# gyuhyun-lee/offline_raytracer

Hardware: AMD Instinct MI355X
Metric: Mpaths/s (higher is better)
Workload: dtype f32; 1 GPU; c3_bunny_room.scn (69451 triangles) 1920x1080 1024spp rr0.8, CHUNK policy chunk=64, one frame sharded in 8x8 blocks over 1 GPU(s); width=1920, height=1080, spp=1024, gather=none (1 GPU): un-permute kernel only, gather_fallback=False, launch=single process, workspace_bytes_per_rank=398131200

## Files before the change

### offline_raytracer_amd/csrc/ort_kernels.hip

```cpp
#include <algorithm>
#include <type_traits>

#include "ort_lane.h"
#include "ort_plan.h"
#include "ort_setup.h"

#ifndef ORT_HOST_SIM
void ort_launch_w5(int diffuse, unsigned int grid, void *stream, const void *sv_bytes, const void *hot_bytes);
size_t ort_w5_sizeof_scene_view();
size_t ort_w5_sizeof_render_hot();
void ort_launch_radiance_adaptive(int counters, int diffuse, int tabs, unsigned int grid, void *stream, const void *sv_bytes, const void *hot_bytes);
size_t ort_adaptive_sizeof_scene_view();
size_t ort_adaptive_sizeof_render_hot();
size_t ort_adaptive_sizeof_render_view();

namespace ort {

using namespace ortd;

static_assert(kPlanBlock == (uint32_t)kBlock && kPlanLdsStack == (uint32_t)kLdsStack && kPlanStashVecs == kStashVecs && kPlanCapL == kCapL &&
              kPlanCapR == kCapR && (int)PLAN_JOBS_EXPLICIT == (int)JOBS_EXPLICIT &&
              (int)PLAN_JOBS_PIXEL == (int)JOBS_PIXEL && (int)PLAN_JOBS_CHUNK == (int)JOBS_CHUNK,
              "ort_plan.h counts with the lane code's limits");

// ... 353 lines not shown
        fprintf(stderr, "  %g ms: %zu", m, n);
    }
    fprintf(stderr, "\n");
    return ORT_OK;
}

static int print_util_diag(const DeviceScene *d, std::string *err) {
    static const char *names[8] = {"node visit", "leaf visit", "traverse outer iteration", "shade call", "  of which lanes with a finished ray",
                                   "produce_ray pass", "  bounce draw", "  sin/cos + ray setup"};
    unsigned long long u[16];
    ORT_HIP(hipMemcpy(u, d->ctrl() + 8, sizeof(u), hipMemcpyDeviceToHost));
    for (int k = 0; k < 8; ++k)
        fprintf(stderr, "util %-40s wave-events %14llu  mean active lanes %6.2f\n", names[k], u[2 * k],
                u[2 * k] ? (double)u[2 * k + 1] / (double)u[2 * k] : 0.0);
    static const char *pnames[10] = {"resolve_hit (chain check)", "hit processing + bounce draw", "pixel / job / new sample", "sin/cos + normalise + ray setup",
                                    "1/d + analytic prologue", "descend loop", "leaf", "pt_lane loop top (after traverse)",
                                    "produce_ray entry (after resolve)", "traverse loop top"};
    unsigned long long ph[30];
    ORT_HIP(hipMemcpy(ph, d->ctrl() + 8 + 32, sizeof(ph), hipMemcpyDeviceToHost));
    double total = 0;
    for (int k = 0; k < 10; ++k) total += (double)ph[3 * k];
    for (int k = 0; k < 10; ++k)
        fprintf(stderr, "phase %-36s share %5.1f %%  cycles/mark %8.1f  marks %12llu  lanes at mark %5.1f\n", pnames[k],
                total > 0 ? 100.0 * (double)ph[3 * k] / total : 0.0, ph[3 * k + 1] ? (double)ph[3 * k] / (double)ph[3 * k + 1] : 0.0,
                ph[3 * k + 1], ph[3 * k + 1] ? (double)ph[3 * k + 2] / (double)ph[3 * k + 1] : 0.0);
    return ORT_OK;
}

static int read_render_stats(const DeviceScene *d, bool counters, ort_stats *stats, std::string *err) {
    memset(stats, 0, sizeof(*stats));
    float ms = 0;
    ORT_HIP(hipEventElapsedTime(&ms, d->ev0, d->ev1));
    stats->kernel_ms = ms;
    unsigned long long c[6];
    ORT_HIP(hipMemcpy(c, d->ctrl() + 1, sizeof(c), hipMemcpyDeviceToHost));
    stats->fallback_rays = c[5];
    if (counters) { stats->paths = c[0]; stats->rays = c[1]; stats->node_tests = c[2]; stats->tri_tests = c[3]; stats->analytic_tests = c[4]; }
    return ORT_OK;
}

int device_render(Scene *scene, const ort_render_params *p, const ort_tile_job *jobs, uint32_t job_count, void *d_out,
                  float *h_out, void *stream_v, uint32_t *final_states, ort_stats *stats, std::string *err, const ort_view *views,
                  uint32_t view_count) {
    DeviceScene *d = scene->dev;
    if (!d) { *err = "scene is not uploaded to a device (ort_scene_upload)"; return ORT_ERR_NO_DEVICE; }
    ORT_HIP(hipSetDevice(d->device));
    hipStream_t stream = (hipStream_t)stream_v;
    const bool packed_out = (p->flags & ORT_RENDER_PACKED) != 0 && !jobs;
    if (!views) view_count = 1;
    const size_t image_bytes = packed_out ? (size_t)block_grid_for(p).my_blocks * 768u : (size_t)view_count * (size_t)p->width * (size_t)p->height * 12u;
    int rc;
    if ((rc = settle_inflight(d, err))) return rc;

    float *out = (float *)d_out;
    if (!out) {
        if ((rc = d->staging.ensure(image_bytes, err))) return rc;
        out = d->staging.as<float>();
        if (h_out) ORT_HIP(hipMemcpyAsync(out, h_out, image_bytes, hipMemcpyHostToDevice, stream));
    }

    SceneView sv = scene_view(scene, d);
    const bool w5_layout_ok = ort_w5_sizeof_scene_view() == sizeof(SceneView) && ort_w5_sizeof_render_hot() == sizeof(RenderHot);
    const LaunchPlan pl = plan_render(scene_traits(scene, d), *p, jobs != nullptr, job_count, w5_layout_ok, d->knobs, view_count);

    sv.util = pl.util ? d->ctrl() + 8 : nullptr;
    if (pl.wide) sv.nodes = d->nodes4.as<const float4>();
    ort_camera cam;
    camera_basis(*scene, p->width, p->height, &cam);
    if (views && !pl.views) cam = views[0].camera;
    memcpy(sv.cam, &cam, sizeof(cam));

    RenderView rv{};
    rv.W = p->width; rv.H = p->height;
    rv.x0 = p->x0; rv.y0 = p->y0; rv.x1 = p->x1; rv.y1 = p->y1;
    rv.seed = views && !pl.views ? views[0].seed : p->seed; rv.spp = p->spp; rv.chunk = p->chunk; rv.rr = p->rr;
    rv.out = out;
    rv.packed_out = packed_out;
    rv.next_job = d->ctrl();
    rv.counters = d->ctrl() + 1;
    rv.mode = pl.mode; rv.nchunks = pl.nchunks; rv.job_count = pl.job_count;
    rv.shard_count = pl.blocks.shard_count; rv.shard_index = pl.blocks.shard_index;
    rv.blocks_w = pl.blocks.blocks_w; rv.block_x0 = pl.blocks.block_x0; rv.block_y0 = pl.blocks.block_y0;
    rv.my_blocks = pl.blocks.my_blocks;
    rv.refill_below = pl.refill_below; rv.descend_below = pl.descend_below;
    rv.capL = pl.capL; rv.capR = pl.capR;
    rv.long_min = pl.long_min; rv.long_refill = pl.long_refill; rv.inflight_cap = pl.inflight_cap; rv.park_min = pl.park_min;
    rv.endgame_from = pl.endgame_from;
    rv.stash_wave_f4 = pl.stash_wave_f4;
    rv.block_major = pl.block_major;
    rv.job_batch = pl.job_batch; rv.batch_until = pl.batch_until;

    if (jobs) {
        if ((rc = d->jobs.ensure((size_t)job_count * sizeof(ort_tile_job), err))) return rc;
        ORT_HIP(hipStreamSynchronize(stream));
        ORT_HIP(hipMemcpy(d->jobs.p, jobs, (size_t)job_count * sizeof(ort_tile_job), hipMemcpyHostToDevice));
        rv.jobs = d->jobs.as<const ort_tile_job>();
        if (final_states) {
            if ((rc = d->states.ensure((size_t)job_count * 4u, err))) return rc;
            rv.final_states = d->states.as<uint32_t>();
        }
    }
    if (pl.views) {
        std::vector<float> &tab = d->view_tab_host;
        pack_view_table(views, view_count, tab);
        if ((rc = d->view_tab.ensure(tab.size() * sizeof(float), err))) return rc;
        ORT_HIP(hipMemcpyAsync(d->view_tab.p, tab.data(), tab.size() * sizeof(float), hipMemcpyHostToDevice, stream));
        rv.views = d->view_tab.as<const float4>();
        rv.view_jobs = pl.view_jobs;
        rv.view_count = pl.view_count;
    }
    if (pl.mode == PLAN_JOBS_CHUNK) {
        if ((rc = d->partial.ensure(pl.partial_bytes, err))) return rc;
        rv.partial = d->partial.as<float>();
    }
    if (pl.exchange) {
        if ((rc = d->stash.ensure(pl.stash_bytes, err))) return rc;
        rv.stash = d->stash.as<float4>();
    }
    ORT_HIP(hipMemsetAsync(d->ctrl(), 0, 128 * sizeof(unsigned long long), stream));
    if (pl.drain_bytes && stats) {
        if ((rc = d->drain.ensure(pl.drain_bytes, err))) return rc;
        ORT_HIP(hipMemsetAsync(d->drain.p, 0, pl.drain_bytes, stream));
        rv.drain = d->drain.as<unsigned long long>();
    }
    ORT_HIP(hipMemcpyAsync(d->rv_dev.p, &rv, sizeof(RenderView), hipMemcpyHostToDevice, stream));
    const RenderHot hot = render_hot<RenderHot>(rv, d->rv_dev.p);
    if (stats) ORT_HIP(hipEventRecord(d->ev0, stream));
    if (pl.wavefront) rc = pl.counters ? launch_wavefront<true>(d, sv, rv, hot, stream, err) : launch_wavefront<false>(d, sv, rv, hot, stream, err);
    else rc = launch_path_tracer(pl, stream, sv, hot, err);
    if (rc) return rc;
    ORT_HIP(hipGetLastError());
    if (rv.mode == JOBS_CHUNK) {
        unsigned long long total = (unsigned long long)rv.my_blocks * 64ull;
        unsigned int cgrid = (unsigned int)((total + 255) / 256);
        if (pl.views) {
            cgrid = (unsigned int)((total * pl.view_count + 255) / 256);
            if (cgrid) hipLaunchKernelGGL(combine_chunks_views, dim3(cgrid), dim3(256), 0, stream, hot);
        } else if (cgrid) hipLaunchKernelGGL(combine_chunks, dim3(cgrid), dim3(256), 0, stream, hot);
        ORT_HIP(hipGetLastError());
    }
    if (stats) ORT_HIP(hipEventRecord(d->ev1, stream));

    if (!d_out && h_out) ORT_HIP(hipMemcpyAsync(h_out, out, image_bytes, hipMemcpyDeviceToHost, stream));
    if (final_states) ORT_HIP(hipMemcpyAsync(final_states, d->states.p, (size_t)job_count * 4u, hipMemcpyDeviceToHost, stream));
    ORT_HIP(hipEventRecord(d->ev_done, stream));
    d->inflight = true;
    if (stats || !d_out || final_states)
        if ((rc = settle_inflight(d, err, "reference-order fallback queue overflowed"))) return rc;
    if (stats && d->knobs.debug_fallback && (rc = print_fallback_diag(d, pl, err))) return rc;
    if (stats && rv.drain && (rc = print_drain_diag(d, pl, err))) return rc;
    if (stats && (rc = read_render_stats(d, pl.counters, stats, err))) return rc;
    if (stats && pl.counters && pl.util && (rc = print_util_diag(d, err))) return rc;
    return ORT_OK;
}

constexpr uint64_t kRaycastSlice = 1ull << 22;
constexpr uint64_t kRadianceSlice = 1ull << 20;

static int ensure_prim_src(Scene *scene, DeviceScene *d, std::string *err) {
    if (d->prim_src.p) return ORT_OK;
    std::vector<uint32_t> src;
    const bool bijective = invert_prim_slots(scene->tree, d->info_box, d->info_cyl, d->info_sphere, src);
    if (!bijective) { *err = "internal: the tree's slot maps are not a bijection onto its shape arrays"; return ORT_ERR_INTERNAL; }
    return upload_vec(src, &d->prim_src, err);
}

static RaycastIO ray_query_io(Scene *scene, DeviceScene *d, const void *d_rays) {
// ... 187 lines not shown
```

### offline_raytracer_amd/csrc/ort_lane.h

```cpp
#ifndef ORT_LANE_H
#define ORT_LANE_H

#include <hip/hip_runtime.h>

#include <math.h>
#include <stdio.h>
#include <stdlib.h>
#include <string.h>

#include <algorithm>
#include <string>
#include <vector>

#include "ort_device.h"
#include "ort_scene.h"
#include "ort_setup.h"

#ifdef ORT_W5_TU
#define ORT_NS ort_w5
#elif defined(ORT_ADAPTIVE_TU)
#define ORT_NS ort_ad
#else
#define ORT_NS ort
#endif
// ... 33 lines not shown
    uint32_t bfs_queue_cap, bfs_queue_count;
    unsigned long long *fallback_counters;
};

struct PrimInfo { uint32_t chain, mat; };

struct SceneView {
    const float4 *tab_src;
    uint32_t tab_flags;
    const float4 *nodes;
    const float4 *tris;
    const float4 *spheres;
    const float4 *boxes;
    const float4 *cyls;
    const PrimInfo *prim_info;
    uint32_t info_box, info_cyl, info_sphere;
    const float4 *materials;
    const uint32_t *light_is_sphere;
    uint32_t light_count;
    uint32_t pro_boxes, pro_spheres, pro_cyls;
    float cam[12];
    const float4 *chain_boxes;
    const ORT_CONSTANT_AS SceneCold *cold;
    unsigned long long *util;
    uint32_t force_fallback_mask;
};

inline void build_prim_info(const Tree &t, const RefTree &rt, std::vector<PrimInfo> &out, uint32_t &info_box, uint32_t &info_cyl, uint32_t &info_sphere) {
    info_box = (uint32_t)t.tri_mat.size();
    info_cyl = info_box + (uint32_t)t.box_mat.size();
    info_sphere = info_cyl + (uint32_t)t.cyl_mat.size();
    out.assign((size_t)info_sphere + t.sphere_mat.size(), PrimInfo{0u, 0u});
    auto fill = [&out](uint32_t base, const std::vector<uint32_t> &chain, const std::vector<uint32_t> &mat) {
        for (size_t i = 0; i < mat.size(); ++i) out[base + i] = PrimInfo{i < chain.size() ? chain[i] : 0u, mat[i]};
    };
    fill(0u, rt.tri_chain, t.tri_mat);
    fill(info_box, rt.box_chain, t.box_mat);
    fill(info_cyl, rt.cyl_chain, t.cyl_mat);
    fill(info_sphere, rt.sphere_chain, t.sphere_mat);
}

enum : int { JOBS_EXPLICIT = 0, JOBS_PIXEL = 1, JOBS_CHUNK = 2 };

struct RenderView {
    int mode;
    const ort_tile_job *jobs;
    uint32_t *final_states;
    unsigned long long job_count;
    int W, H, x0, y0, x1, y1;
    uint32_t seed, spp, chunk, nchunks;
    float rr;
    int refill_below;
    int descend_below;
    uint32_t shard_index, shard_count, blocks_w, my_blocks;
    uint32_t block_x0, block_y0;
    float *out;
    float *partial;
    int packed_out;
    unsigned long long *next_job;
    unsigned long long *counters;
    float4 *stash;
    uint32_t stash_wave_f4;
    uint32_t capL, capR;
    uint32_t long_min;
    uint32_t long_refill;
    uint32_t park_min;
    uint32_t inflight_cap;
    uint32_t block_major;
    unsigned long long endgame_from;
    uint32_t job_batch;
    unsigned long long batch_until;
    unsigned long long *drain;
    const float4 *views;
    unsigned long long view_jobs;
    uint32_t view_count;
    const float2 *rays;
    const uint32_t *seeds;
    uint32_t ray_tree_spheres, ray_tree_quadrics, ray_tree_boxes;
    float ray_lo[3], ray_hi[3];
    uint32_t ad_min_spp, ad_check_every;
    float ad_tolerance, ad_floor;
    uint32_t *ad_spp;
    float *ad_m2;
};


struct RenderHot {
    int mode, W, H;
    float rr;
    int refill_below, descend_below;
    const ORT_CONSTANT_AS RenderView *c;
};

struct WfView {
    uint32_t slots;
    float4 *od0;
    float2 *od1;
    float4 *hit0;
    uint32_t *hitp;
    float4 *p0;
    float4 *p1;
    float4 *p2;
    uint4 *p3;
    uint32_t *flags;
    unsigned long long *active;
};

enum : int { PS_NEED_JOB = 0, PS_PIXEL = 1, PS_SAMPLE = 2, PS_HIT = 3, PS_DONE = 4 };

#ifdef ORT_HOST_SIM
#define ORT_BALLOT(p) ((p) ? 1ull : 0ull)
#define ORT_POPC64(m) __builtin_popcountll(m)
#define ORT_NEXT_JOB(p) __atomic_fetch_add((p), 1ull, __ATOMIC_RELAXED)
#define ORT_COUNT(p, v) ((void)__atomic_fetch_add((p), (v), __ATOMIC_RELAXED))
#define ORT_TRY_LOCK(p) (*(p) == 0u ? (*(p) = 1u, true) : false)
#define ORT_PEEK(p) (*(p))
#define ORT_BACKOFF()
#define ORT_UNLOCK(p) (*(p) = 0u)
#define ORT_FENCE()
#define ORT_FFS64(m) __builtin_ffsll((long long)(m))
#define ORT_LANE() 0
#define ORT_UTIL(sv, k, pred)
#define ORT_PHASE(pr, sv, k, pred)
#ifndef ORT_SIM_PIXEL_HOOK
#define ORT_SIM_PIXEL_HOOK(x, y, rng)
#endif
#ifndef ORT_SIM_RAY_HOOK
#define ORT_SIM_RAY_HOOK(x, y, o, d, t, n, m)
#endif
#else
#define ORT_SIM_PIXEL_HOOK(x, y, rng)
#define ORT_SIM_RAY_HOOK(x, y, o, d, t, n, m)
#define ORT_BALLOT(p) __ballot(p)
#define ORT_POPC64(m) __popcll(m)
#define ORT_NEXT_JOB(p) atomicAdd((p), 1ull)
#define ORT_COUNT(p, v) atomicAdd((p), (v))
#define ORT_TRY_LOCK(p) (atomicCAS((p), 0u, 1u) == 0u)
#define ORT_PEEK(p) __hip_atomic_load((p), __ATOMIC_RELAXED, __HIP_MEMORY_SCOPE_AGENT)
#define ORT_BACKOFF() __builtin_amdgcn_s_sleep(64)
#define ORT_UNLOCK(p) ((void)atomicExch((p), 0u))
#define ORT_FENCE() __threadfence()
#define ORT_FFS64(m) __ffsll((unsigned long long)(m))
#define ORT_LANE() ((int)__lane_id())
#define ORT_UTIL(sv, k, pred)                                                                        \
    do {                                                                                             \
        if (COUNTERS && (sv).util && blockIdx.x < 32u) {                                             \
            unsigned long long m_ = __ballot(pred);                                                  \
            if (m_ && (int)__lane_id() == __ffsll(m_) - 1) {                                         \
                atomicAdd(&g_lds_prof[2 * (k)], 1ull);                                               \
                atomicAdd(&g_lds_prof[2 * (k) + 1], (unsigned long long)__popcll(m_));               \
            }                                                                                        \
        }                                                                                            \
    } while (0)
#define ORT_PHASE(pr, sv, k, pred)                                                                   \
    do {                                                                                             \
        if (COUNTERS && (pr).on) {                                                                   \
            const unsigned long long now_ = __builtin_amdgcn_s_memtime();                            \
            const unsigned long long m_ = __ballot(pred), a_ = __ballot(true);                       \
             \
            unsigned long long *last_ = &g_lds_prof[96 + (threadIdx.x >> 6)];                        \
            if ((int)__lane_id() == __ffsll(a_) - 1) {                                               \
                atomicAdd(&g_lds_prof[32 + 3 * (k)], now_ - *last_);                                 \
                atomicAdd(&g_lds_prof[32 + 3 * (k) + 1], 1ull);                                      \
                atomicAdd(&g_lds_prof[32 + 3 * (k) + 2], (unsigned long long)__popcll(m_));          \
                *last_ = __builtin_amdgcn_s_memtime();                                               \
            }                                                                                        \
// ... 888 lines not shown
    float t0y = (a.y - org.y) * inv_d.y, t1y = (b.x - org.y) * inv_d.y;
    float t0z = (a.z - org.z) * inv_d.z, t1z = (b.y - org.z) * inv_d.z;
    float n0 = fmaxf(fmaxf(fminf(t0x, t1x), fminf(t0y, t1y)), fminf(t0z, t1z));
    float f0 = fminf(fminf(fmaxf(t0x, t1x), fmaxf(t0y, t1y)), fmaxf(t0z, t1z));
    float u0x = (b.z - org.x) * inv_d.x, u1x = (cc.y - org.x) * inv_d.x;
    float u0y = (b.w - org.y) * inv_d.y, u1y = (cc.z - org.y) * inv_d.y;
    float u0z = (cc.x - org.z) * inv_d.z, u1z = (cc.w - org.z) * inv_d.z;
    float n1 = fmaxf(fmaxf(fminf(u0x, u1x), fminf(u0y, u1y)), fminf(u0z, u1z));
    float f1 = fminf(fminf(fmaxf(u0x, u1x), fmaxf(u0y, u1y)), fmaxf(u0z, u1z));
    bool h0 = (f0 * 1.0000004f >= n0) && (f0 >= 0.0f) && ((n0 * kCullSlack < best_t) || (c0 & SPHERE_BELOW_BIT));
    bool h1 = (f1 * 1.0000004f >= n1) && (f1 >= 0.0f) && ((n1 * kCullSlack < best_t) || (c1 & SPHERE_BELOW_BIT)) && (c1 != EMPTY_CHILD);
    if (h0 && h1) {
        bool swap = n1 < n0;
        uint32_t farc = swap ? c0 : c1;
        cur = swap ? c1 : c0;
        if (sp < LDS_ENTRIES) lds_stack[sp * BLOCK + tid] = farc;
        else spill[sp - LDS_ENTRIES] = farc;
        sp++;
    } else if (h0) {
        cur = c0;
    } else if (h1) {
        cur = c1;
    } else if (sp == 0) {
        cur = kTraversalDone;
    } else {
        sp--;
        if (sp < LDS_ENTRIES) cur = lds_stack[sp * BLOCK + tid];
        else cur = ((volatile uint32_t *)spill)[sp - LDS_ENTRIES];
    }
}

template <bool COUNTERS, int LDS_ENTRIES, int BLOCK>
ORT_D void visit_node4(float4 lx, float4 ly, float4 lz, float4 hx, float4 hy, float4 hz, float4 cw, V3 org, V3 inv_d, float best_t, uint32_t &cur, int &sp,
                       uint32_t *lds_stack, uint32_t *spill, int tid, Counters &c) {
    if (COUNTERS) c.nodes += 4;
    float key0, key1, key2, key3;
    uint32_t w0, w1, w2, w3;
#define ORT_SLAB4(K, W, LX, LY, LZ, HX, HY, HZ, CW)                                                                        \
    {                                                                                                                      \
        const float t0x = ((LX) - org.x) * inv_d.x, t1x = ((HX) - org.x) * inv_d.x;                                        \
        const float t0y = ((LY) - org.y) * inv_d.y, t1y = ((HY) - org.y) * inv_d.y;                                        \
        const float t0z = ((LZ) - org.z) * inv_d.z, t1z = ((HZ) - org.z) * inv_d.z;                                        \
        const float n_ = fmaxf(fmaxf(fminf(t0x, t1x), fminf(t0y, t1y)), fminf(t0z, t1z));                                  \
        const float f_ = fminf(fminf(fmaxf(t0x, t1x), fmaxf(t0y, t1y)), fmaxf(t0z, t1z));                                  \
        const uint32_t cw_ = om_f32_bits(CW);                                                                              \
        const bool hit_ = (f_ * 1.0000004f >= n_) && (f_ >= 0.0f) && ((n_ * kCullSlack < best_t) || (cw_ & SPHERE_BELOW_BIT)) && (cw_ != EMPTY_CHILD); \
        K = hit_ ? fminf(n_, 3.402823466e+38f) : __builtin_inff();              \
        W = hit_ ? cw_ : EMPTY_CHILD;                                                                                      \
    }
    ORT_SLAB4(key0, w0, lx.x, ly.x, lz.x, hx.x, hy.x, hz.x, cw.x)
    ORT_SLAB4(key1, w1, lx.y, ly.y, lz.y, hx.y, hy.y, hz.y, cw.y)
    ORT_SLAB4(key2, w2, lx.z, ly.z, lz.z, hx.z, hy.z, hz.z, cw.z)
    ORT_SLAB4(key3, w3, lx.w, ly.w, lz.w, hx.w, hy.w, hz.w, cw.w)
#undef ORT_SLAB4
#define ORT_CX(KA, WA, KB, WB)                                                                                             \
    {                                                                                                                      \
        const bool sw_ = KB < KA;                                                                                          \
        const float ka_ = sw_ ? KB : KA, kb_ = sw_ ? KA : KB;                                                              \
        const uint32_t wa_ = sw_ ? WB : WA, wb_ = sw_ ? WA : WB;                                                           \
        KA = ka_; KB = kb_; WA = wa_; WB = wb_;                                                                            \
    }
    ORT_CX(key0, w0, key1, w1)
    ORT_CX(key2, w2, key3, w3)
    ORT_CX(key0, w0, key2, w2)
    ORT_CX(key1, w1, key3, w3)
    ORT_CX(key1, w1, key2, w2)
#undef ORT_CX
    if (w0 == EMPTY_CHILD) {
        if (sp == 0) {
            cur = kTraversalDone;
        } else {
            sp--;
            if (sp < LDS_ENTRIES) cur = lds_stack[sp * BLOCK + tid];
            else cur = ((volatile uint32_t *)spill)[sp - LDS_ENTRIES];
        }
        return;
    }
    cur = w0;
    if (w3 != EMPTY_CHILD) { if (sp < LDS_ENTRIES) lds_stack[sp * BLOCK + tid] = w3; else spill[sp - LDS_ENTRIES] = w3; sp++; }
    if (w2 != EMPTY_CHILD) { if (sp < LDS_ENTRIES) lds_stack[sp * BLOCK + tid] = w2; else spill[sp - LDS_ENTRIES] = w2; sp++; }
    if (w1 != EMPTY_CHILD) { if (sp < LDS_ENTRIES) lds_stack[sp * BLOCK + tid] = w1; else spill[sp - LDS_ENTRIES] = w1; sp++; }
}

template <bool COUNTERS, bool TABS, int LDS_ENTRIES, int BLOCK>
ORT_D void begin_ray(const SceneView &sv, const float4 *tab, const PathState &P, Trav &T, HitState &h, Counters &c, Prof &pr,
                     uint32_t *lds_stack, uint32_t *spill, int tid) {
    T.cur = 0;
    T.sp = 0;
    T.inv_d = mk(1.0f / P.dir.x, 1.0f / P.dir.y, 1.0f / P.dir.z);
    reset_hit(h, 3.402823466e+38f);
    prologue_tests<COUNTERS, TABS>(sv, tab, P.org, P.dir, T.inv_d, h, c);
    ORT_PHASE(pr, sv, 4, true);
}

template <bool COUNTERS, int LDS_ENTRIES, int BLOCK, bool TREELET = false, bool ANNOUNCE = false, bool WIDE = false>
ORT_D bool traverse(const SceneView &sv, V3 org, V3 dir, Trav &T, HitState &h, uint32_t *lds_stack, uint32_t *spill, int tid,
                    int refill_below, int descend_below, Counters &c, Prof &pr, uint32_t excl = kNoPrim, const float4 *tab = nullptr) {
    bool tracing = true;
    uint32_t cur = T.cur;
    int sp = T.sp;
    const V3 inv_d = T.inv_d;
    while (tracing) {
        ORT_UTIL(sv, 2, true);
        ORT_PHASE(pr, sv, 9, true);
        const int entering = ORT_POPC64(ORT_BALLOT((cur & LEAF_BIT) == 0u));
        const int stragglers = descend_below < (entering >> ORT_DESCEND_SHIFT) ? descend_below : (entering >> ORT_DESCEND_SHIFT);
        while (!(cur & LEAF_BIT)) {
            ORT_UTIL(sv, 0, true);
            const uint32_t ni = cur & NODE_INDEX_MASK;
            if (WIDE) {
                const float4 *np = sv.nodes + 8u * ni;
                const float4 lx = np[0], ly = np[1], lz = np[2], hx = np[3], hy = np[4], hz = np[5], cw = np[6];
                visit_node4<COUNTERS, LDS_ENTRIES, BLOCK>(lx, ly, lz, hx, hy, hz, cw, org, inv_d, h.best_t, cur, sp, lds_stack, spill, tid, c);
            } else {
            float4 na, nb, nc, nd;
            if (TREELET && ni < kTreeletNodes) {
                const float4 *np = tab + kTabTreelet + 4u * ni;
                na = np[0]; nb = np[1]; nc = np[2]; nd = np[3];
            } else {
                const float4 *np = sv.nodes + 4u * ni;
                na = np[0]; nb = np[1]; nc = np[2]; nd = np[3];
            }
            visit_node<COUNTERS, LDS_ENTRIES, BLOCK>(na, nb, nc, nd, org, inv_d, h.best_t, cur, sp, lds_stack, spill, tid, c);
            }
            if (ORT_POPC64(ORT_BALLOT(true)) < stragglers) break;
        }
        ORT_PHASE(pr, sv, 5, true);
        if (!(cur & LEAF_BIT)) {
        } else if (cur == kTraversalDone) {
            tracing = false;
        } else {
            ORT_UTIL(sv, 1, true);
            uint32_t kind = (cur >> 28) & 7u, count = ((cur >> 24) & 15u) + 1u, first = cur & 0x00ffffffu;
            for (uint32_t i = 0; i < count; ++i)
                test_prim<COUNTERS, false>(sv, kind, first + i, org, dir, inv_d, h.best_t, h.hit_n, h.hit_prim, h.phantom_t, h.runner_t, c.tris, c.analytic, excl);
            if (sp == 0) {
                cur = kTraversalDone;
                tracing = false;
            } else {
                sp--;
                if (sp < LDS_ENTRIES) cur = lds_stack[sp * BLOCK + tid];
                else cur = ((volatile uint32_t *)spill)[sp - LDS_ENTRIES];
            }
            ORT_PHASE(pr, sv, 6, true);
        }
        if (ANNOUNCE && !tracing) announce_winner<BLOCK>(sv, h.hit_prim, lds_stack, tid);
        if (refill_below > 0 && ORT_POPC64(ORT_BALLOT(tracing)) < refill_below) break;
    }
    T.cur = cur;
    T.sp = sp;
    return tracing;
}

template <bool COUNTERS, bool TABS, int LDS_ENTRIES, int BLOCK, bool ANNOUNCED = false, bool WIDE = false>
ORT_D void resolve_hit(const SceneView &sv, const float4 *tab, V3 org, V3 dir, V3 inv_d, uint32_t lane_id, HitState &h, Counters &c, Prof &pr,
                       uint32_t *lds_stack, uint32_t *spill, int tid) {
    uint32_t word = 0, mat = 0;
    if (ANNOUNCED) {
        announced_info<BLOCK>(lds_stack, tid, word, mat);
    } else if (h.hit_prim != kNoPrim) {
        const PrimInfo pi = sv.prim_info[info_index(sv, h.hit_prim)];
        word = pi.chain; mat = pi.mat;
    }
    bool stale = false;
    bool recast = sv.force_fallback_mask != 0xffffffffu && (om_f32_bits(dir.x) & sv.force_fallback_mask) == 0u;
    if (!ORT_RARE(recast)) {
        if (ORT_RARE(h.phantom_t <= h.best_t)) {
            recast = true;
            ORT_STAT(2, 1);
        } else if (h.hit_prim != kNoPrim) {
            float gap = 0.0f;
            const int verdict = chain_verdict(sv, word, org, inv_d, h.best_t, fminf(h.runner_t, h.phantom_t), gap);
            if (ORT_RARE(verdict != CH_ADMIT)) {
                stale = true;
                ORT_STAT(3, verdict == CH_REJECT ? 0 : 1); ORT_STAT(3, 4 + (int)(h.hit_prim >> 28));
                ORT_COUNT(sv.cold->fallback_counters + kDiagFallback + 1, 1ull);
                const uint32_t w_prim = h.hit_prim;
                uint32_t *save = lds_stack + tid;
                save[(LDS_ENTRIES - 1) * BLOCK] = om_f32_bits(h.best_t);
                save[(LDS_ENTRIES - 2) * BLOCK] = om_f32_bits(h.hit_n.x);
                save[(LDS_ENTRIES - 3) * BLOCK] = om_f32_bits(h.hit_n.y);
                save[(LDS_ENTRIES - 4) * BLOCK] = om_f32_bits(h.hit_n.z);
                Trav t2;
                t2.cur = 0; t2.sp = 0; t2.inv_d = inv_d;
                reset_hit(h, verdict == CH_REJECT ? 3.402823466e+38f : om_bits_f32(om_f32_bits(gap) + 1u));
                prologue_tests<COUNTERS, TABS, true>(sv, tab, org, dir, inv_d, h, c, w_prim);
                (void)traverse<COUNTERS, LDS_ENTRIES - 4, BLOCK, false, false, WIDE>(sv, org, dir, t2, h, lds_stack, spill, tid, 0, 0, c, pr, w_prim);
                if (verdict == CH_UNKNOWN) {
                    if (h.hit_prim != kNoPrim || h.phantom_t <= gap) {
                        recast = true;
                        ORT_STAT(2, h.hit_prim != kNoPrim ? 2 : 6);
                    } else {
                        h.best_t = om_bits_f32(save[(LDS_ENTRIES - 1) * BLOCK]);
                        h.hit_n = mk(om_bits_f32(save[(LDS_ENTRIES - 2) * BLOCK]), om_bits_f32(save[(LDS_ENTRIES - 3) * BLOCK]),
                                     om_bits_f32(save[(LDS_ENTRIES - 4) * BLOCK]));
                        h.hit_prim = w_prim;
                    }
                } else if (h.phantom_t <= h.best_t) {
                    recast = true;
                    ORT_STAT(2, 3);
                } else if (h.hit_prim != kNoPrim) {
                    float gap2 = 0.0f;
                    if (chain_verdict(sv, sv.prim_info[info_index(sv, h.hit_prim)].chain, org, inv_d, h.best_t, fminf(h.runner_t, h.phantom_t), gap2) != CH_ADMIT) { recast = true; ORT_STAT(2, 4); }
                }
            }
        }
    }
    recast_exactly<COUNTERS>(sv, recast, org, dir, inv_d, lane_id, h, c);
    if (ORT_RARE(stale || recast)) mat = (h.hit_prim != kNoPrim) ? sv.prim_info[info_index(sv, h.hit_prim)].mat : 0u;
    h.hit_mat = (h.hit_prim != kNoPrim) ? mat : 0u;
}

ORT_D void flush_counters(const RenderHot &rv, const Counters &c, bool all) {
    if (all) {
        ORT_COUNT(rv.c->counters + 0, c.paths);
        ORT_COUNT(rv.c->counters + 1, c.rays);
        ORT_COUNT(rv.c->counters + 2, c.nodes);
        ORT_COUNT(rv.c->counters + 3, c.tris);
        ORT_COUNT(rv.c->counters + 4, c.analytic);
    }
}

template <bool COUNTERS, bool DIFFUSE = false, bool TABS = false, bool IMPLICIT = false, bool WIDE = false, bool VIEWS = false>
ORT_D void pt_lane(const SceneView &sv, const RenderHot &rv, const float4 *tab, uint32_t *lds_stack, float *lds_focal, const int tid,
                   const uint32_t lane_id, bool prof_on = false, unsigned long long *pool = nullptr) {
    uint32_t spill[kSpillStack];
    const uint32_t spp_u = IMPLICIT ? ((rv.mode == JOBS_PIXEL) ? rv.c->spp : rv.c->chunk) : 0u;
    Prof pr;
    pr.on = prof_on;
#ifndef ORT_HOST_SIM
    if (COUNTERS && prof_on) pr.t = __builtin_amdgcn_s_memtime();
#endif
    PathState P;
    HitState h;
    Trav T;
    Counters c;
    bool tracing = false;
    for (;;) {
        if (!tracing) {
            ORT_UTIL(sv, 3, true);
            ORT_UTIL(sv, 4, P.ps == PS_HIT);
            ORT_PHASE(pr, sv, 7, true);
            if (P.ps == PS_HIT) resolve_hit<COUNTERS, TABS, kLdsStack, kBlock, true, WIDE>(sv, tab, P.org, P.dir, T.inv_d, lane_id, h, c, pr, lds_stack, spill, tid);
            ORT_PHASE(pr, sv, 0, P.ps == PS_HIT);
            tracing = produce_ray<COUNTERS, DIFFUSE, TABS, IMPLICIT, VIEWS>(sv, rv, tab, P, h, c, pr, lds_focal + tid, kBlock, spp_u, nullptr, false, pool);
            if (tracing) {
                begin_ray<COUNTERS, TABS, kLdsStack, kBlock>(sv, tab, P, T, h, c, pr, lds_stack, spill, tid);
                if (COUNTERS) c.rays++;
            }
        }
        if (ORT_BALLOT(P.ps != PS_DONE) == 0ull) break;
        if (tracing) tracing = traverse<COUNTERS, kLdsStack, kBlock, TABS && !WIDE, true, WIDE>(sv, P.org, P.dir, T, h, lds_stack, spill, tid, rv.refill_below, rv.descend_below, c, pr, kNoPrim, tab);
    }
    flush_counters(rv, c, COUNTERS);
}


#ifndef ORT_HOST_SIM
struct Stash {
    float4 *rec;
    uint32_t *stk;
    uint32_t cap;
};

ORT_D uint32_t lane_rank(unsigned long long mask) {
    return __builtin_amdgcn_mbcnt_hi((uint32_t)(mask >> 32), __builtin_amdgcn_mbcnt_lo((uint32_t)mask, 0u));
}

constexpr uint32_t kStashVecs = 9u;
constexpr uint32_t kCapL = 128u, kCapR = 192u;
static_assert(kLdsStack % 4 == 0, "the L stash carves its stack words out of float4 units (kLdsStack / 4 per parked path)");
ORT_D void stash_store(const Stash &st, uint32_t slot, const PathState &P, const HitState &h, uint32_t cur, int sp, V3 inv_d, const float *focal_cache,
                       uint32_t info_chain = 0u, uint32_t info_mat = 0u) {
    float4 *r = st.rec + slot;
    const uint32_t cap = st.cap;
    r[0] = make_float4(P.org.x, P.org.y, P.org.z, P.dir.x);
    r[cap] = make_float4(P.dir.y, P.dir.z, h.best_t, om_bits_f32(h.hit_prim));
    r[2u * cap] = make_float4(h.hit_n.x, h.hit_n.y, h.hit_n.z, h.phantom_t);
    r[3u * cap] = make_float4(h.runner_t, om_bits_f32(cur), om_bits_f32((uint32_t)sp), om_bits_f32(P.rng));
    r[4u * cap] = make_float4(P.color.x, P.color.y, P.color.z, P.weight.x);
    r[5u * cap] = make_float4(P.weight.y, P.weight.z, P.wo.x, P.wo.y);
    r[6u * cap] = make_float4(P.wo.z, om_bits_f32(P.pxy), om_bits_f32(P.jyp), om_bits_f32(P.sample | (P.primary ? 0x80000000u : 0u)));
    r[7u * cap] = make_float4(inv_d.x, inv_d.y, inv_d.z, focal_cache[0]);
    r[8u * cap] = make_float4(focal_cache[kBlock], focal_cache[2 * kBlock], om_bits_f32(info_chain), om_bits_f32(info_mat));
}

ORT_D void stash_load(const Stash &st, uint32_t slot, const RenderHot &rv, PathState &P, HitState &h, Trav &T, float *focal_cache, uint32_t *lds_info) {
    const float4 *r = st.rec + slot;
    const uint32_t cap = st.cap;
    const float4 a = r[0], b = r[cap], c = r[2u * cap], d = r[3u * cap], e = r[4u * cap], f = r[5u * cap], g = r[6u * cap];
    const float4 i = r[7u * cap], j = r[8u * cap];
    P.org = mk(a.x, a.y, a.z); P.dir = mk(a.w, b.x, b.y);
    h.best_t = b.z; h.hit_prim = om_f32_bits(b.w);
    h.hit_n = mk(c.x, c.y, c.z); h.phantom_t = c.w;
    h.runner_t = d.x; T.cur = om_f32_bits(d.y); T.sp = (int)om_f32_bits(d.z); P.rng = om_f32_bits(d.w);
    P.color = mk(e.x, e.y, e.z); P.weight = mk(e.w, f.x, f.y); P.wo = mk(f.z, f.w, g.x);
    P.pxy = om_f32_bits(g.y); P.jyp = om_f32_bits(g.z);
    const uint32_t sm = om_f32_bits(g.w);
    P.sample = sm & 0x7fffffffu; P.primary = (sm >> 31) != 0u;
    P.ps = PS_HIT;
    T.inv_d = mk(i.x, i.y, i.z);
    focal_cache[0] = i.w; focal_cache[kBlock] = j.x; focal_cache[2 * kBlock] = j.y;
    lds_info[0] = om_f32_bits(j.z); lds_info[kBlock] = om_f32_bits(j.w);
}

template <bool COUNTERS, bool DIFFUSE, bool TABS>
ORT_D void pt_lane_x(const SceneView &sv, const RenderHot &rv, const float4 *tab, uint32_t *lds_stack, float *lds_focal, const int tid,
                     const uint32_t lane_id, bool prof_on, unsigned long long *pool) {
    uint32_t spill[kSpillStack];
    Prof pr;
    pr.on = prof_on;
    if (COUNTERS && prof_on) pr.t = __builtin_amdgcn_s_memtime();
    PathState P;
    HitState h;
    Trav T;
    Counters c;
    bool tracing = false;

    const uint32_t wave = (uint32_t)__builtin_amdgcn_readfirstlane((int)(lane_id >> 6));
    const uint32_t spp_u = (rv.mode == JOBS_PIXEL) ? rv.c->spp : rv.c->chunk;
    float4 *wbase = rv.c->stash + (size_t)wave * rv.c->stash_wave_f4;
    Stash L, R;
    L.rec = wbase; L.cap = kCapL;
    L.stk = (uint32_t *)(wbase + kStashVecs * kCapL);
    R.rec = wbase + (kStashVecs + (uint32_t)kLdsStack / 4u) * kCapL; R.cap = kCapR; R.stk = nullptr;
    uint32_t ltop = 0, rtop = 0;
    float *focal_cache = lds_focal + tid;
    uint32_t *late_flag = (uint32_t *)lds_focal + 3 * kBlock + tid;
    *late_flag = 0u;
    bool early_end = false;

    for (;;) {
        if (!early_end) early_end = __ballot(*(volatile uint32_t *)late_flag != 0u) != 0ull;
        const unsigned long long m_tr = __ballot(tracing);
        const unsigned long long m_done = __ballot(!tracing && P.ps == PS_HIT);
// ... 615 lines not shown
```

### offline_raytracer_amd/csrc/ort_plan.h

```cpp
#ifndef ORT_PLAN_H
#define ORT_PLAN_H

#include <stddef.h>
#include <stdint.h>
#include <stdlib.h>
#include <string.h>

#include "../../include/ort.h"

namespace ort {

struct Knobs {
    uint32_t force_fallback_mask = 0xffffffffu;
    bool debug_util = false, debug_fallback = false, debug_drain = false;
    int cache_resident = -1;
    int refill_below = -1, descend_below = -1;
    bool wavefront = false;
    bool general_kernel = false;
    int lds_tables = -1;
    int exchange = -1;
    int long_min = -1, long_refill = -1, inflight_cap = -1, park_min = -1;
    int lpt = -1;
    int wide = -1;
    int waves5 = -1;
    int endgame_jobs = -1;
    int blocks_per_cu = -1;
    int job_batch = -1, batch_tail = -1;
};
inline int env_int(const char *name, int unset = -1) {
    const char *e = getenv(name);
    return e ? atoi(e) : unset;
}
inline Knobs read_knobs() {
    Knobs k;
    const char *e;
    if ((e = getenv("ORT_DEBUG_FORCE_FALLBACK"))) k.force_fallback_mask = (uint32_t)strtoul(e, nullptr, 0);
    k.debug_util = getenv("ORT_DEBUG_UTIL") != nullptr;
    k.debug_fallback = getenv("ORT_DEBUG_FALLBACK") != nullptr;
    k.debug_drain = getenv("ORT_DEBUG_DRAIN") != nullptr;
    k.cache_resident = env_int("ORT_CACHE_RESIDENT");
    k.refill_below = env_int("ORT_REFILL_BELOW");
    k.descend_below = env_int("ORT_DESCEND_BELOW");
    k.wavefront = (e = getenv("ORT_MODE")) && strcmp(e, "wavefront") == 0;
    k.general_kernel = (e = getenv("ORT_KERNEL")) && strcmp(e, "general") == 0;
    k.lds_tables = env_int("ORT_LDS_TABLES");
    k.exchange = env_int("ORT_EXCHANGE");
    k.long_min = env_int("ORT_LONG_MIN");
    k.long_refill = env_int("ORT_LONG_REFILL");
    k.inflight_cap = env_int("ORT_INFLIGHT_CAP");
    k.park_min = env_int("ORT_PARK_MIN");
    k.lpt = env_int("ORT_LPT");
    k.wide = env_int("ORT_WIDE");
    k.waves5 = env_int("ORT_WAVES5");
    k.endgame_jobs = env_int("ORT_ENDGAME_JOBS");
    k.blocks_per_cu = env_int("ORT_BLOCKS_PER_CU");
    k.job_batch = env_int("ORT_JOB_BATCH");
    k.batch_tail = env_int("ORT_BATCH_TAIL");
    return k;
}

constexpr uint32_t kPlanBlock = 256;
constexpr uint32_t kPlanLdsStack = 24;
constexpr uint32_t kPlanStashVecs = 9, kPlanCapL = 128, kPlanCapR = 192;
constexpr uint32_t kPlanTabPro = 1u, kPlanTabLights = 2u, kPlanTabMats = 8u;
constexpr uint32_t kPlanAllTabs = kPlanTabPro | kPlanTabLights | kPlanTabMats;
constexpr uint32_t kPlanTabMatCap = 48, kPlanTabLightCap = 64, kPlanTabProCap = 40;
enum : int { PLAN_JOBS_EXPLICIT = 0, PLAN_JOBS_PIXEL = 1, PLAN_JOBS_CHUNK = 2 };

inline unsigned int persistent_blocks(int cu_count, unsigned int per_cu) { return (unsigned int)(cu_count > 0 ? cu_count : 256) * per_cu; }
inline unsigned int upload_max_blocks(int cu_count, const Knobs &kn) {
    unsigned int per_cu = kn.blocks_per_cu > 0 ? (unsigned int)kn.blocks_per_cu : 4u;
    if (per_cu < 1u || per_cu > 8u) per_cu = 4u;
    return persistent_blocks(cu_count, per_cu);
}

inline bool tree_is_cache_resident(size_t fast_tree_bytes, int knob) {
    return knob >= 0 ? knob != 0 : fast_tree_bytes <= (size_t)(16u << 20);
}

struct BlockGrid { uint32_t blocks_w, block_x0, block_y0, my_blocks, shard_index, shard_count; };
inline BlockGrid block_grid_for(const ort_render_params *p) {
    BlockGrid g;
    g.shard_count = p->shard_count > 1 ? p->shard_count : 1;
    g.shard_index = p->shard_count > 1 ? p->shard_index : 0;
    g.blocks_w = (uint32_t)((p->width + 7) / 8);
    uint32_t total = g.blocks_w * (uint32_t)((p->height + 7) / 8);
    g.block_x0 = g.block_y0 = 0;
    if (g.shard_count == 1 && p->x1 > p->x0 && p->y1 > p->y0) {
        g.block_x0 = (uint32_t)(p->x0 / 8);
        g.block_y0 = (uint32_t)(p->y0 / 8);
        g.blocks_w = (uint32_t)((p->x1 + 7) / 8) - g.block_x0;
        total = g.blocks_w * ((uint32_t)((p->y1 + 7) / 8) - g.block_y0);
    }
    g.my_blocks = (total > g.shard_index) ? (total - g.shard_index + g.shard_count - 1) / g.shard_count : 0;
    return g;
}

inline uint64_t shard_block_count(const ort_render_params *p) { return block_grid_for(p).my_blocks; }

inline uint64_t render_workspace_bytes(const ort_render_params *p) {
    if (p->policy != ORT_POLICY_CHUNK || p->chunk == 0) return 0;
    uint64_t nch = p->spp / p->chunk;
    return nch * (uint64_t)block_grid_for(p).my_blocks * 64ull * 12ull;
}
inline uint64_t render_views_workspace_bytes(const ort_render_params *p, uint32_t view_count) { return (uint64_t)view_count * render_workspace_bytes(p); }

inline uint32_t table_fit_flags(size_t material_count, size_t light_count, uint32_t pro_boxes, uint32_t pro_spheres, uint32_t pro_cyls) {
    uint32_t flags = 0;
    if (2ull * pro_boxes + pro_spheres + 4ull * pro_cyls <= kPlanTabProCap) flags |= kPlanTabPro;
    if (light_count <= kPlanTabLightCap) flags |= kPlanTabLights;
    if (material_count <= kPlanTabMatCap) flags |= kPlanTabMats;
    return flags;
}

struct SceneTraits {
    bool diffuse_only = false;
    uint32_t tab_flags = 0;
    size_t fast_tree_bytes = 0;
    float sah_cost = 0;
    bool has_wide = false;
    int cu_count = 0;
    unsigned int max_blocks = 0;
};

inline void plan_loop_exits(bool cache_resident_tree, const Knobs &kn, int *refill_below, int *descend_below) {
    *refill_below = kn.refill_below >= 0 ? kn.refill_below : (cache_resident_tree ? 16 : 32);
    if (*refill_below < 1) *refill_below = 1;
    if (*refill_below > 64) *refill_below = 64;
    *descend_below = kn.descend_below >= 0 ? kn.descend_below : (cache_resident_tree ? 8 : 16);
    if (*descend_below < 0) *descend_below = 0;
    if (*descend_below > 64) *descend_below = 64;
}

inline void plan_job_batches(unsigned long long job_count, unsigned long long lanes, const Knobs &kn, uint32_t *job_batch, unsigned long long *batch_until) {
    *job_batch = kn.job_batch >= 0 ? (uint32_t)kn.job_batch : (job_count >= 96ull * lanes ? 128u : 64u);
    const unsigned long long per_lane = kn.batch_tail >= 0 ? (unsigned long long)kn.batch_tail : 8ull * ((*job_batch + 63u) / 64u);
    const unsigned long long tail = per_lane * lanes;
    *batch_until = job_count > tail ? job_count - tail : 0ull;
}

struct LaunchPlan {
    bool wavefront = false, exchange = false, five = false, wide = false, counters = false, diffuse = false, tabs = false, implicit = false;
    bool util = false;
    bool views = false;
    uint32_t view_count = 1;
    unsigned long long view_jobs = 0;
    unsigned int grid = 1;
    int mode = PLAN_JOBS_EXPLICIT;
    uint32_t nchunks = 0;
    unsigned long long job_count = 0;
    BlockGrid blocks{};
    int refill_below = 0, descend_below = 0;
    uint32_t capL = 0, capR = 0, long_min = 0, long_refill = 0, inflight_cap = 0, park_min = 0;
    unsigned long long endgame_from = 0;
    uint32_t stash_wave_f4 = 0;
    uint32_t block_major = 0;
    uint32_t job_batch = 0;
    unsigned long long batch_until = 0;
    size_t partial_bytes = 0, stash_bytes = 0, drain_bytes = 0;
};

inline LaunchPlan plan_render(const SceneTraits &t, const ort_render_params &p, bool explicit_jobs, uint64_t job_count, bool w5_layout_ok,
                              const Knobs &kn, uint32_t view_count = 1) {
    LaunchPlan pl;
    const bool views = view_count > 1u && !explicit_jobs;
    const bool want_util = kn.debug_util && !views;
    const bool cache_resident_tree = tree_is_cache_resident(t.fast_tree_bytes, kn.cache_resident);
    plan_loop_exits(cache_resident_tree, kn, &pl.refill_below, &pl.descend_below);

    pl.blocks = block_grid_for(&p);
    if (explicit_jobs) {
        pl.mode = PLAN_JOBS_EXPLICIT;
        pl.job_count = job_count;
    } else if (p.policy == ORT_POLICY_PIXEL) {
        pl.mode = PLAN_JOBS_PIXEL;
        pl.nchunks = 1;
        pl.job_count = (unsigned long long)pl.blocks.my_blocks * 64ull;
    } else {
        pl.mode = PLAN_JOBS_CHUNK;
        pl.nchunks = p.spp / p.chunk;
        pl.job_count = (unsigned long long)pl.blocks.my_blocks * 64ull * pl.nchunks;
        pl.partial_bytes = (size_t)pl.nchunks * (size_t)pl.blocks.my_blocks * 64u * 12u;
    }
    pl.view_jobs = pl.job_count;
    if (views) {
        pl.views = true;
        pl.view_count = view_count;
        pl.job_count *= view_count;
        pl.partial_bytes *= view_count;
    }

    const bool counters = (p.flags & ORT_RENDER_COUNTERS) != 0;
    const bool wavefront = kn.wavefront && !views;
    const bool diffuse = t.diffuse_only && !kn.general_kernel;
    const bool tabs = (t.tab_flags & kPlanAllTabs) == kPlanAllTabs && kn.lds_tables != 0;
    const bool can_five = !views && !wavefront && !counters && tabs && pl.mode != PLAN_JOBS_EXPLICIT && kn.wide <= 0 && kn.exchange <= 0 && w5_layout_ok;
    unsigned long long lanes_wanted = pl.job_count;
    unsigned int max_blocks = t.max_blocks;
    unsigned int grid = (unsigned int)((lanes_wanted + kPlanBlock - 1) / kPlanBlock);
    if (grid > max_blocks) grid = max_blocks;
    if (grid == 0) grid = 1;
    bool exch = false;
    if (!wavefront) {
        const bool worth_it = diffuse && cache_resident_tree && t.sah_cost >= 0.09f && pl.job_count >= 24ull * (unsigned long long)grid * kPlanBlock;
        exch = !views && tabs && pl.mode != PLAN_JOBS_EXPLICIT && (kn.exchange >= 0 ? kn.exchange != 0 : worth_it) && (!counters || (want_util && diffuse));
        if (exch && kn.refill_below < 0) pl.refill_below = 24;
        if (exch) {
            pl.capL = kPlanCapL; pl.capR = kPlanCapR;
            pl.long_min = kn.long_min >= 0 ? (uint32_t)kn.long_min : 64u;
            pl.long_refill = kn.long_refill >= 0 ? (uint32_t)kn.long_refill : 32u;
            pl.inflight_cap = kn.inflight_cap >= 0 ? (uint32_t)kn.inflight_cap : 64u;
            pl.park_min = kn.park_min >= 0 ? (uint32_t)kn.park_min : 1u;
            if (pl.long_min < 1u) pl.long_min = 1u;
            if (pl.long_min > pl.capL) pl.long_min = pl.capL;
            if (pl.long_refill > 64u) pl.long_refill = 64u;
            if (pl.inflight_cap < pl.long_min) pl.inflight_cap = pl.long_min;
            if (pl.inflight_cap < 1u) pl.inflight_cap = 1u;
            {
                const unsigned long long quarter_jobs = kn.endgame_jobs >= 0 ? (unsigned long long)kn.endgame_jobs : 16ull;
                const unsigned long long tail_jobs = quarter_jobs * (unsigned long long)grid * kPlanBlock / 4ull;
                pl.endgame_from = pl.job_count > tail_jobs ? pl.job_count - tail_jobs : 0ull;
            }
            pl.stash_wave_f4 = (kPlanStashVecs + kPlanLdsStack / 4u) * pl.capL + kPlanStashVecs * pl.capR;
            pl.stash_bytes = (size_t)t.max_blocks * (kPlanBlock / 64) * pl.stash_wave_f4 * 16u;
        }
    }
    const bool five = can_five && !exch && (kn.waves5 >= 0 ? kn.waves5 != 0 : (!diffuse || !cache_resident_tree));
    if (five && kn.blocks_per_cu <= 0) {
        max_blocks = persistent_blocks(t.cu_count, 5u);
        grid = (unsigned int)((lanes_wanted + kPlanBlock - 1) / kPlanBlock);
        if (grid > max_blocks) grid = max_blocks;
        if (grid == 0) grid = 1;
    }
    if (pl.mode == PLAN_JOBS_CHUNK && pl.nchunks >= 2u && kn.lpt != 0) pl.block_major = 1u;
    if (!wavefront) plan_job_batches(pl.job_count, (unsigned long long)grid * kPlanBlock, kn, &pl.job_batch, &pl.batch_until);
    if (kn.debug_drain && !wavefront) pl.drain_bytes = (size_t)max_blocks * (kPlanBlock / 64) * sizeof(unsigned long long);
    const bool wide = !views && t.has_wide && !exch && tabs && (counters || pl.mode != PLAN_JOBS_EXPLICIT) && !(counters && diffuse && want_util) && kn.wide > 0;

    pl.wavefront = wavefront;
    pl.counters = counters;
    pl.util = want_util;
    pl.exchange = exch;
    pl.five = five;
    pl.wide = wide && !wavefront;
    pl.diffuse = diffuse && (!counters || want_util);
    pl.tabs = tabs;
    pl.implicit = !wavefront && !counters && tabs && pl.mode != PLAN_JOBS_EXPLICIT;
    pl.grid = grid;
    return pl;
}

struct QueryPlan {
    bool counters = false, diffuse = false, tabs = false;
    unsigned int grid = 1;
    int refill_below = 0, descend_below = 0;
    uint32_t job_batch = 0;
    unsigned long long batch_until = 0;
};

inline unsigned int query_grid(const SceneTraits &t, uint64_t count) {
    const uint64_t blocks = (count + kPlanBlock - 1) / kPlanBlock;
    return (unsigned int)(blocks < t.max_blocks ? blocks : t.max_blocks);
}

#ifndef ORT_RAYCAST_REFILL
#define ORT_RAYCAST_REFILL 32
#endif
#ifndef ORT_RAYCAST_BATCH
#define ORT_RAYCAST_BATCH 1024
#endif
#ifndef ORT_RAYCAST_TAIL
#define ORT_RAYCAST_TAIL 4
#endif
inline QueryPlan plan_ray_query(const SceneTraits &t, uint64_t count, bool counters) {
    QueryPlan pl;
    pl.counters = counters;
    pl.tabs = (t.tab_flags & kPlanTabPro) != 0;
    pl.grid = query_grid(t, count);
    const unsigned long long lanes = (unsigned long long)pl.grid * kPlanBlock;
    pl.refill_below = ORT_RAYCAST_REFILL;
    pl.descend_below = tree_is_cache_resident(t.fast_tree_bytes, -1) ? 8 : 16;
    pl.job_batch = ORT_RAYCAST_BATCH;
    pl.batch_until = count > ORT_RAYCAST_TAIL * lanes ? count - ORT_RAYCAST_TAIL * lanes : 0ull;
    return pl;
}

inline QueryPlan plan_radiance(const SceneTraits &t, uint64_t count, bool counters, const Knobs &kn) {
    QueryPlan pl;
    plan_loop_exits(tree_is_cache_resident(t.fast_tree_bytes, kn.cache_resident), kn, &pl.refill_below, &pl.descend_below);
    pl.counters = counters;
    pl.diffuse = t.diffuse_only && !kn.general_kernel;
    pl.tabs = (t.tab_flags & kPlanAllTabs) == kPlanAllTabs && kn.lds_tables != 0;
    pl.grid = query_grid(t, count);
    if (pl.grid == 0) pl.grid = 1;
    plan_job_batches(count, (unsigned long long)pl.grid * kPlanBlock, kn, &pl.job_batch, &pl.batch_until);
    return pl;
}

}

#endif
```

Measured before the change: 5184 Mpaths/s.

## Visit BVH root in begin_ray and gate traversal entry on wave occupancy

begin_ray now tests the root node (wide or binary) right after producing a ray, so rays that miss the root finish without entering the traversal loop. The traversal call is also gated by a ballot: a wave enters traverse only when at least traverse_min lanes are tracing or when they are half of the live lanes. With the default traverse_min of 1 the gate always passes whenever any lane is tracing, so only the root pre-visit changes behaviour by default. The aim is to lower divergence and loop overhead in the persistent lane kernel, at the cost of an extra ballot and popcount per iteration and more code in begin_ray.

```diff
diff --git a/offline_raytracer_amd/csrc/ort_kernels.hip b/offline_raytracer_amd/csrc/ort_kernels.hip
--- a/offline_raytracer_amd/csrc/ort_kernels.hip
+++ b/offline_raytracer_amd/csrc/ort_kernels.hip
@@ -459,7 +459,7 @@
     rv.shard_count = pl.blocks.shard_count; rv.shard_index = pl.blocks.shard_index;
     rv.blocks_w = pl.blocks.blocks_w; rv.block_x0 = pl.blocks.block_x0; rv.block_y0 = pl.blocks.block_y0;
     rv.my_blocks = pl.blocks.my_blocks;
-    rv.refill_below = pl.refill_below; rv.descend_below = pl.descend_below;
+    rv.refill_below = pl.refill_below; rv.descend_below = pl.descend_below; rv.traverse_min = pl.traverse_min;
     rv.capL = pl.capL; rv.capR = pl.capR;
     rv.long_min = pl.long_min; rv.long_refill = pl.long_refill; rv.inflight_cap = pl.inflight_cap; rv.park_min = pl.park_min;
     rv.endgame_from = pl.endgame_from;
diff --git a/offline_raytracer_amd/csrc/ort_lane.h b/offline_raytracer_amd/csrc/ort_lane.h
--- a/offline_raytracer_amd/csrc/ort_lane.h
+++ b/offline_raytracer_amd/csrc/ort_lane.h
@@ -139,6 +139,7 @@
     float ad_tolerance, ad_floor;
     uint32_t *ad_spp;
     float *ad_m2;
+    int traverse_min;
 };
 
 
@@ -1193,15 +1194,33 @@
     if (w1 != EMPTY_CHILD) { if (sp < LDS_ENTRIES) lds_stack[sp * BLOCK + tid] = w1; else spill[sp - LDS_ENTRIES] = w1; sp++; }
 }
 
-template <bool COUNTERS, bool TABS, int LDS_ENTRIES, int BLOCK>
-ORT_D void begin_ray(const SceneView &sv, const float4 *tab, const PathState &P, Trav &T, HitState &h, Counters &c, Prof &pr,
+template <bool COUNTERS, bool TABS, int LDS_ENTRIES, int BLOCK, bool ROOT = false, bool WIDE = false>
+ORT_D bool begin_ray(const SceneView &sv, const float4 *tab, const PathState &P, Trav &T, HitState &h, Counters &c, Prof &pr,
                      uint32_t *lds_stack, uint32_t *spill, int tid) {
     T.cur = 0;
     T.sp = 0;
     T.inv_d = mk(1.0f / P.dir.x, 1.0f / P.dir.y, 1.0f / P.dir.z);
     reset_hit(h, 3.402823466e+38f);
     prologue_tests<COUNTERS, TABS>(sv, tab, P.org, P.dir, T.inv_d, h, c);
+    bool tracing = true;
+    if constexpr (ROOT) {
+        ORT_UTIL(sv, 0, true);
+        if constexpr (WIDE) {
+            const float4 *np = sv.nodes;
+            const float4 lx = np[0], ly = np[1], lz = np[2], hx = np[3], hy = np[4], hz = np[5], cw = np[6];
+            visit_node4<COUNTERS, LDS_ENTRIES, BLOCK>(lx, ly, lz, hx, hy, hz, cw, P.org, T.inv_d, h.best_t, T.cur, T.sp, lds_stack, spill, tid, c);
+        } else {
+            const float4 *np = TABS ? tab + kTabTreelet : sv.nodes;
+            const float4 na = np[0], nb = np[1], nc = np[2], nd = np[3];
+            visit_node<COUNTERS, LDS_ENTRIES, BLOCK>(na, nb, nc, nd, P.org, T.inv_d, h.best_t, T.cur, T.sp, lds_stack, spill, tid, c);
+        }
+        if (T.cur == kTraversalDone) {
+            tracing = false;
+            announce_winner<BLOCK>(sv, h.hit_prim, lds_stack, tid);
+        }
+    }
     ORT_PHASE(pr, sv, 4, true);
+    return tracing;
 }
 
 template <bool COUNTERS, int LDS_ENTRIES, int BLOCK, bool TREELET = false, bool ANNOUNCE = false, bool WIDE = false>
@@ -1347,6 +1366,7 @@
     Trav T;
     Counters c;
     bool tracing = false;
+    const int traverse_min = rv.c->traverse_min;
     for (;;) {
         if (!tracing) {
             ORT_UTIL(sv, 3, true);
@@ -1354,14 +1374,16 @@
             ORT_PHASE(pr, sv, 7, true);
             if (P.ps == PS_HIT) resolve_hit<COUNTERS, TABS, kLdsStack, kBlock, true, WIDE>(sv, tab, P.org, P.dir, T.inv_d, lane_id, h, c, pr, lds_stack, spill, tid);
             ORT_PHASE(pr, sv, 0, P.ps == PS_HIT);
-            tracing = produce_ray<COUNTERS, DIFFUSE, TABS, IMPLICIT, VIEWS>(sv, rv, tab, P, h, c, pr, lds_focal + tid, kBlock, spp_u, nullptr, false, pool);
-            if (tracing) {
-                begin_ray<COUNTERS, TABS, kLdsStack, kBlock>(sv, tab, P, T, h, c, pr, lds_stack, spill, tid);
+            if (produce_ray<COUNTERS, DIFFUSE, TABS, IMPLICIT, VIEWS>(sv, rv, tab, P, h, c, pr, lds_focal + tid, kBlock, spp_u, nullptr, false, pool)) {
+                tracing = begin_ray<COUNTERS, TABS, kLdsStack, kBlock, true, WIDE>(sv, tab, P, T, h, c, pr, lds_stack, spill, tid);
                 if (COUNTERS) c.rays++;
             }
         }
-        if (ORT_BALLOT(P.ps != PS_DONE) == 0ull) break;
-        if (tracing) tracing = traverse<COUNTERS, kLdsStack, kBlock, TABS && !WIDE, true, WIDE>(sv, P.org, P.dir, T, h, lds_stack, spill, tid, rv.refill_below, rv.descend_below, c, pr, kNoPrim, tab);
+        const unsigned long long live = ORT_BALLOT(P.ps != PS_DONE);
+        if (live == 0ull) break;
+        const int waiting = ORT_POPC64(ORT_BALLOT(tracing));
+        const bool enter = waiting >= traverse_min || 2 * waiting >= ORT_POPC64(live);
+        if (tracing && enter) tracing = traverse<COUNTERS, kLdsStack, kBlock, TABS && !WIDE, true, WIDE>(sv, P.org, P.dir, T, h, lds_stack, spill, tid, rv.refill_below, rv.descend_below, c, pr, kNoPrim, tab);
     }
     flush_counters(rv, c, COUNTERS);
 }
diff --git a/offline_raytracer_amd/csrc/ort_plan.h b/offline_raytracer_amd/csrc/ort_plan.h
--- a/offline_raytracer_amd/csrc/ort_plan.h
+++ b/offline_raytracer_amd/csrc/ort_plan.h
@@ -15,6 +15,7 @@
     bool debug_util = false, debug_fallback = false, debug_drain = false;
     int cache_resident = -1;
     int refill_below = -1, descend_below = -1;
+    int traverse_min = -1;
     bool wavefront = false;
     bool general_kernel = false;
     int lds_tables = -1;
@@ -41,6 +42,7 @@
     k.cache_resident = env_int("ORT_CACHE_RESIDENT");
     k.refill_below = env_int("ORT_REFILL_BELOW");
     k.descend_below = env_int("ORT_DESCEND_BELOW");
+    k.traverse_min = env_int("ORT_TRAVERSE_MIN");
     k.wavefront = (e = getenv("ORT_MODE")) && strcmp(e, "wavefront") == 0;
     k.general_kernel = (e = getenv("ORT_KERNEL")) && strcmp(e, "general") == 0;
     k.lds_tables = env_int("ORT_LDS_TABLES");
@@ -132,6 +134,15 @@
     if (*descend_below > 64) *descend_below = 64;
 }
 
+inline int plan_traverse_min(bool five, bool diffuse, bool cache_resident_tree, const Knobs &kn) {
+    int v = 1;
+    (void)five; (void)diffuse; (void)cache_resident_tree;
+    if (kn.traverse_min >= 0) v = kn.traverse_min;
+    if (v < 1) v = 1;
+    if (v > 64) v = 64;
+    return v;
+}
+
 inline void plan_job_batches(unsigned long long job_count, unsigned long long lanes, const Knobs &kn, uint32_t *job_batch, unsigned long long *batch_until) {
     *job_batch = kn.job_batch >= 0 ? (uint32_t)kn.job_batch : (job_count >= 96ull * lanes ? 128u : 64u);
     const unsigned long long per_lane = kn.batch_tail >= 0 ? (unsigned long long)kn.batch_tail : 8ull * ((*job_batch + 63u) / 64u);
@@ -151,6 +162,7 @@
     unsigned long long job_count = 0;
     BlockGrid blocks{};
     int refill_below = 0, descend_below = 0;
+    int traverse_min = 1;
     uint32_t capL = 0, capR = 0, long_min = 0, long_refill = 0, inflight_cap = 0, park_min = 0;
     unsigned long long endgame_from = 0;
     uint32_t stash_wave_f4 = 0;
@@ -237,6 +249,8 @@
     if (kn.debug_drain && !wavefront) pl.drain_bytes = (size_t)max_blocks * (kPlanBlock / 64) * sizeof(unsigned long long);
     const bool wide = !views && t.has_wide && !exch && tabs && (counters || pl.mode != PLAN_JOBS_EXPLICIT) && !(counters && diffuse && want_util) && kn.wide > 0;
 
+    pl.traverse_min = plan_traverse_min(five, diffuse, cache_resident_tree, kn);
+
     pl.wavefront = wavefront;
     pl.counters = counters;
     pl.util = want_util;
```

Result: slower. 4658 Mpaths/s (-10.1%).
